# artpixls/ART

Measured on AMD Instinct MI355X. Metric: megapixels/sec end-to-end (AMaZE+FTblockDN+tone), 45 MP Bayer, higher is better.
Workload: dtype f32; 1 GPU; AMaZE + getImage/matrix + ImProcFunctions::denoise (chroma noise-curve map, FTblockDN wavelet shrinkage luma 40 / chroma 15 / gamma 1.7 + DCT detail recovery 50) + exposure 0.3 EV + tone curve STD, 8192x5464 Bayer RGGB fp32, 1 frame per GPU per step (BASELINE configs[2]); frame=8192x5464, lanes_per_gpu=1, parallelism=frame-per-gpu x1, completion_records=1, completion_via=single process

## Files before the change

### art_amd/csrc/detail.hip

```cpp
#include <hip/hip_runtime.h>
#include "devmath.h"
#include "devsleef.h"
#include "dct64.h"
#include "kernels.h"

namespace artgpu {

namespace {
constexpr int TS = 64, OFF = 25, BLKRAD = 1;
constexpr int NXCD = 8;
__device__ __forceinline__ int reflect(int v, int n)
{
    if (v < 0) return -v < n - 1 ? -v : n - 1;
    if (v >= n) return 2 * n - 2 - v > 0 ? 2 * n - 2 - v : 0;
    return v;
}
}

template <int RAD>
__global__ void __launch_bounds__(64) detail_blocks_kernel(DetailArgs a)
{
    constexpr int XR = 4;
    __shared__ float B[TS + XR][TS + 1];
    const int lane = threadIdx.x;
    const int wk = (a.numblox_W + NXCD - 1) / NXCD;
    const int xcd = blockIdx.x % NXCD, idx = blockIdx.x / NXCD;
    const int vblk = idx / wk, hblk = xcd * wk + (idx - vblk * wk);
    if (hblk >= a.numblox_W) return;
    const int blk = vblk * a.numblox_W + hblk;
    const int top = (vblk - BLKRAD) * OFF, left = (hblk - BLKRAD) * OFF;
    constexpr int rad = RAD;
    float x[TS];

    {
        const int cc = reflect(left + lane, a.w);
#pragma unroll
        for (int i = 0; i < TS; ++i) {
            const int rr = reflect(top + i, a.h);
            const size_t o = (size_t)rr * a.w + cc;
            x[i] = a.tm_in[i * TS + lane] * (a.Lin[o] - a.L[o]);
        }
    }
    lee_fwd<TS>(x);
#pragma unroll
    for (int k = 0; k < TS; ++k) B[k][lane] = 2.f * x[k];
    __syncthreads();
#pragma unroll
    for (int j = 0; j < TS; ++j) x[j] = B[lane][j];
    lee_fwd<TS>(x);
#pragma unroll
    for (int m = 0; m < TS; ++m) x[m] = 2.f * x[m];
    {
        int len = rad + 1;
        float tempval = fabsf(x[0]);
#pragma unroll
        for (int q = 1; q <= rad; q++) tempval += fabsf(x[q]);
        tempval /= len;
        B[lane][0] = tempval;
#pragma unroll
        for (int col = 1; col <= rad; col++) {
            tempval = (tempval * len + fabsf(x[col + rad])) / (len + 1);
            B[lane][col] = tempval;
            len++;
        }
        const float rlen = 1.f / (float)len;
#pragma unroll
        for (int col = rad + 1; col < TS - rad; col++) {
            tempval = tempval + (fabsf(x[col + rad]) - fabsf(x[col - rad - 1])) * rlen;
            B[lane][col] = tempval;
        }
#pragma unroll
        for (int col = TS - rad; col < TS; col++) {
            tempval = (tempval * len - fabsf(x[col - rad - 1])) / (len - 1);
            B[lane][col] = tempval;
            len--;
        }
    }
    __syncthreads();
    {
        float lenf = (float)(rad + 1);
        float tv = B[0][lane];
#pragma unroll
        for (int i = 1; i <= rad; i++) tv = tv + B[i][lane];
        tv = tv / lenf;
        const bool colin = (left + lane) >= 0 && (left + lane) < a.w;
        const float inv_hi = 1.f / a.detail_hi, inv_lo = 1.f / a.detail_lo;
        auto emit = [&](int row, float tvr) {
            const bool rowin = (top + row) >= 0 && (top + row) < a.h;
            float factor = (rowin && colin) ? a.detail_hi : a.detail_lo;
            const float rfac = (rowin && colin) ? inv_hi : inv_lo;
            const bool masked = a.mask && rowin && colin;
            if (masked) {
                const float d = a.params_Ldetail * a.mask[(size_t)(top + row) * a.w + left + lane];
                const float t = static_cast<float>((100. - d) * (100. - d) + 50. * (100. - d)) * TS * 0.5f;
                factor = t * t;
            }
            (void)factor; (void)rfac;
            const int slot = row > rad ? row - rad - 1 : TS + row;
#ifdef DETAIL_EXACT_DIV
            B[slot][lane] = 1.0f - __expf(-sqr(tvr) / factor);
#else
            if (a.mask) B[slot][lane] = 1.0f - __expf(masked ? -sqr(tvr) / factor : -sqr(tvr) * rfac);
            else B[slot][lane] = 1.0f - __expf(-sqr(tvr) * rfac);
#endif
        };
        emit(0, tv);
#pragma unroll
        for (int row = 1; row <= rad; ++row) {
            const float lenp1 = lenf + 1.f;
            tv = (tv * lenf + B[row + rad][lane]) / lenp1;
            lenf = lenp1;
            emit(row, tv);
        }
        const float rlen = 1.f / lenf;
        constexpr int S0 = rad + 1, S1 = TS - rad, G = 8;
        constexpr int SG = S0 + (S1 - S0) / G * G;
#ifndef DETAIL_ROW_AT_A_TIME
#pragma unroll 1
        for (int r0 = S0; r0 < SG; r0 += G) {
            float hi[G], lo[G], tvs[G];
#pragma unroll
            for (int k = 0; k < G; ++k) { hi[k] = B[r0 + k + rad][lane]; lo[k] = B[r0 + k - rad - 1][lane]; }
#pragma unroll
            for (int k = 0; k < G; ++k) { tv = tv + (hi[k] - lo[k]) * rlen; tvs[k] = tv; }
#pragma unroll
            for (int k = 0; k < G; ++k) emit(r0 + k, tvs[k]);
        }
#pragma unroll 1
        for (int row = SG; row < S1; ++row) {
#else
#pragma unroll 1
        for (int row = S0; row < S1; ++row) {
#endif
            tv = tv + (B[row + rad][lane] - B[row - rad - 1][lane]) * rlen;
            emit(row, tv);
        }
#pragma unroll 1
        for (int row = S1; row < TS; ++row) {
            const float lenm1 = lenf - 1.f;
            tv = (tv * lenf - B[row - rad - 1][lane]) / lenm1;
            lenf = lenm1;
            emit(row, tv);
        }
    }
    __syncthreads();
    {
        const int slot = lane > rad ? lane - rad - 1 : TS + lane;
#pragma unroll
        for (int m = 0; m < TS; ++m) x[m] = x[m] * B[slot][m];
    }
    __syncthreads();
#pragma unroll
    for (int m = 1; m < TS; ++m) x[m] = 2.f * x[m];
    lee_inv<TS>(x);
#pragma unroll
    for (int j = 0; j < TS; ++j) B[lane][j] = x[j];
    __syncthreads();
    x[0] = B[0][lane];
#pragma unroll
    for (int k = 1; k < TS; ++k) x[k] = 2.f * B[k][lane];
    lee_inv<TS>(x);
    float *out = a.blocks + (size_t)blk * TS * TS;
#pragma unroll
    for (int i = 0; i < TS; ++i) out[i * TS + lane] = x[i];
}

__global__ void __launch_bounds__(1024) detail_gather_kernel(DetailArgs a)
{
    __shared__ float s_in[TS * TS], s_out[TS * TS];
    for (int k = threadIdx.x; k < TS * TS; k += 1024) { s_in[k] = a.tm_in[k]; s_out[k] = a.tm_out[k]; }
    __syncthreads();
    const float DCTnorm = 1.0f / (4 * TS * TS);
    const long long n = (long long)a.w * a.h;
#ifndef DETAIL_GATHER_LOOPS
    for (long long t = blockIdx.x * (long long)blockDim.x + threadIdx.x; t < n; t += (long long)gridDim.x * blockDim.x) {
        const int y = (int)(t / a.w), x = (int)(t - (long long)y * a.w);
        const int yc = y / OFF, xc = x / OFF, ry = y - yc * OFF, rx = x - xc * OFF;
        bool vs[3], hs[3];
        int iv[3], jh[3], vb[3], hb[3];
#pragma unroll
        for (int k = 0; k < 3; ++k) {
            vs[k] = k > 0 || (yc > 0 && ry < TS - 2 * OFF);
            hs[k] = k > 0 || (xc > 0 && rx < TS - 2 * OFF);
            iv[k] = vs[k] ? ry + 2 * OFF - OFF * k : ry;  vb[k] = vs[k] ? yc - 1 + k : yc + 1;
            jh[k] = hs[k] ? rx + 2 * OFF - OFF * k : rx;  hb[k] = hs[k] ? xc - 1 + k : xc + 1;
        }
        float blk[9], tmo[9], tmi[9];
#pragma unroll
        for (int s_ = 0; s_ < 3; ++s_)
#pragma unroll
            for (int t_ = 0; t_ < 3; ++t_) {
                const int m = iv[s_] * TS + jh[t_];
                blk[3 * s_ + t_] = a.blocks[((size_t)vb[s_] * a.numblox_W + hb[t_]) * TS * TS + m];
                tmo[3 * s_ + t_] = s_out[m];
                tmi[3 * s_ + t_] = s_in[m];
            }
        const float Lold = a.L[t];
// ... 1 lines not shown
#pragma unroll
        for (int s_ = 0; s_ < 3; ++s_)
#pragma unroll
            for (int t_ = 0; t_ < 3; ++t_) {
                const bool v = vs[s_] && hs[t_];
                const float ld = Ldetail + tmo[3 * s_ + t_] * blk[3 * s_ + t_] * DCTnorm, tw = totwt + tmi[3 * s_ + t_] * tmo[3 * s_ + t_];
                Ldetail = v ? ld : Ldetail;
                totwt = v ? tw : totwt;
            }
        a.L[t] = Lold + Ldetail / totwt;
    }
#else
    for (long long t = blockIdx.x * (long long)blockDim.x + threadIdx.x; t < n; t += (long long)gridDim.x * blockDim.x) {
        const int y = (int)(t / a.w), x = (int)(t - (long long)y * a.w);
        const int vb0 = max(0, y / OFF + BLKRAD - 2), vb1 = min(a.numblox_H - 1, y / OFF + BLKRAD);
        const int hb0 = max(0, x / OFF + BLKRAD - 2), hb1 = min(a.numblox_W - 1, x / OFF + BLKRAD);
        float Ldetail = 0.f, totwt = 0.f;
        for (int vblk = vb0; vblk <= vb1; ++vblk) {
            const int i = y - (vblk - BLKRAD) * OFF;
            if (i < 0 || i >= TS) continue;
            for (int hblk = hb0; hblk <= hb1; ++hblk) {
                const int j = x - (hblk - BLKRAD) * OFF;
                if (j < 0 || j >= TS) continue;
                const float tmo = s_out[i * TS + j];
                Ldetail += tmo * a.blocks[((size_t)vblk * a.numblox_W + hblk) * TS * TS + i * TS + j] * DCTnorm;
                totwt += s_in[i * TS + j] * tmo;
            }
        }
        a.L[t] += Ldetail / totwt;
    }
#endif
}

hipError_t launch_detail_blocks(const DetailArgs &a, hipStream_t s)
{
    const dim3 grid(NXCD * ((a.numblox_W + NXCD - 1) / NXCD) * a.numblox_H);
    switch (a.blur_rad) {
    case 1: hipLaunchKernelGGL(detail_blocks_kernel<1>, grid, dim3(64), 0, s, a); break;
    case 2: hipLaunchKernelGGL(detail_blocks_kernel<2>, grid, dim3(64), 0, s, a); break;
    case 3: hipLaunchKernelGGL(detail_blocks_kernel<3>, grid, dim3(64), 0, s, a); break;
    default: return hipErrorInvalidValue;
    }
    return hipGetLastError();
}
hipError_t launch_detail_gather(const DetailArgs &a, hipStream_t s)
{
    const long long n = (long long)a.w * a.h;
    const long long g = (n + 1023) / 1024;
    int dev = 0, cus = 256;
    if (hipGetDevice(&dev) == hipSuccess) (void)hipDeviceGetAttribute(&cus, hipDeviceAttributeMultiprocessorCount, dev);
    const long long cap = 2LL * cus;
    hipLaunchKernelGGL(detail_gather_kernel, dim3((int)(g < cap ? g : cap)), dim3(1024), 0, s, a);
    return hipGetLastError();
}

}
```

### art_amd/csrc/artgpu_api.hip

```cpp
#include <hip/hip_runtime.h>
#include <dlfcn.h>
#include <cmath>
#include <cstdio>
#include <cstdarg>
#include <cstring>
#include <new>
#include <string>
#include <thread>
#include <vector>
#include <algorithm>

#include "../../include/artgpu.h"
#include "kernels.h"

using namespace artgpu;

struct artgpu_ctx {
    int device = 0;
    hipStream_t stream = nullptr;
    hipStream_t aux = nullptr;
    hipEvent_t aux_ev[2] = {nullptr, nullptr};
    hipStream_t dn_stream[1] = {nullptr};
    hipEvent_t dn_ev[2] = {nullptr, nullptr};
    const float *gam_tab = nullptr; float gam_key[6] = {};
    int opt_lut_lds = 1;
    int opt_dn_streams = 0;
    int ccalc_nonneg = 0;
    int opt_dn_fused = 1;
    std::string err;
    int *fs_diag = nullptr;
    int opt_dn_debug_stall = -1;
    long opt_dn_wait_ms = 0;
    long long batch_px = 0;
    int dn_form = -1, dn_form_streak = 0;
    float *arena = nullptr;
    size_t arena_bytes = 0;
    static constexpr int NSTAGE = 8;
    float *stage[NSTAGE] = {};
    size_t stage_bytes[NSTAGE] = {};
    static constexpr int NPOOL = 64;
    float *pool[NPOOL] = {};
    size_t pool_bytes[NPOOL] = {};
    std::vector<artgpu_ctx *> lanes;
    int batch_lanes = 1;
    int frames_in_flight = 1;
    bool owns_stream = false;
    hipStream_t io_up = nullptr, io_down = nullptr;
    hipEvent_t io_ev[8] = {};
    int *io_host = nullptr;
    int io_host_cap = 0;
    int cu_reserve = 0;
    int opt_io_direct = -1;
    float fuse_pre = 0.f, fuse_post = 0.f;
    GetImageFuse fuse_gi = {};
    float fuse_exp_scale = 0.f, fuse_exp_black = 0.f;
    int fuse_exp_on = 0;
    int tail_exp_on = 0;
    float tail_exp_scale = 0.f, tail_exp_black = 0.f;
    float *bbox = nullptr;
    size_t bbox_bytes = 0;
    float *amz_lists = nullptr;
// ... 354 lines not shown
}

int artgpu_get_option(artgpu_ctx *ctx, const char *name, long *value)
{
    if (!ctx || !name || !value) return ARTGPU_EINVAL;
    const std::string n(name);
    if (n.rfind("amaze_counter", 0) == 0 && n.size() == 14 && n[13] >= '0' && n[13] <= '7') {
        if (!ctx->amz_lists || ctx->amz_nstream <= 0) { *value = 0; return ARTGPU_OK; }
        HIPCHK(ctx, hipSetDevice(ctx->device));
        HIPCHK(ctx, hipStreamSynchronize(ctx->stream));
        const size_t nfixed = (((size_t)ctx->amz_nstream + (1 + ctx->amz_narena) + (1 + ctx->amz_narena + ctx->amz_nstream) + 3) / 4) * 4;
        int v = 0;
        HIPCHK(ctx, hipMemcpy(&v, reinterpret_cast<int *>(ctx->amz_lists) + nfixed + 4 + 2 * (size_t)ctx->amz_nstream + (n[13] - '0'), sizeof(int), hipMemcpyDeviceToHost));
        *value = v;
        return ARTGPU_OK;
    }
    return fail(ctx, ARTGPU_EINVAL, "get_option: unknown option '%s'", name);
}

int artgpu_set_option(artgpu_ctx *ctx, const char *name, long value)
{
    if (!ctx || !name) return ARTGPU_EINVAL;
    const std::string n(name);
    if (n == "amaze_path") { if (value < 0 || value > 1) return fail(ctx, ARTGPU_EINVAL, "amaze_path: 0 or 1"); ctx->opt_amaze_path = (int)value; }
    else if (n == "amaze_split") ctx->opt_amaze_split = value != 0;
    else if (n == "amaze_overlap") ctx->opt_amaze_overlap = value != 0;
    else if (n == "amaze_grid") { if (value < 0) return fail(ctx, ARTGPU_EINVAL, "amaze_grid: >= 0"); ctx->opt_amaze_grid = (int)value; }
    else if (n == "amaze_zero_mask") ctx->opt_amaze_zero_mask = value;
    else if (n == "amaze_zero_frame") ctx->opt_amaze_zero_frame = (int)value;
    else if (n == "amaze_poison") ctx->opt_amaze_poison = (int)value;
    else if (n == "roctx") ctx->opt_roctx = value != 0;
    else if (n == "dn_streams") ctx->opt_dn_streams = value != 0;
    else if (n == "dn_fused") ctx->opt_dn_fused = (int)value;
    else if (n == "dn_debug_stall") ctx->opt_dn_debug_stall = (int)value;
    else if (n == "dn_wait_ms") ctx->opt_dn_wait_ms = value < 0 ? 0 : value;
    else if (n == "lut_lds") ctx->opt_lut_lds = value != 0;
    else if (n == "cu_reserve") { if (value < 0 || value > 4096) return fail(ctx, ARTGPU_EINVAL, "cu_reserve: 0 .. 4096"); ctx->cu_reserve = (int)value; }
    else if (n == "io_direct") { if (value < -1 || value > 4096) return fail(ctx, ARTGPU_EINVAL, "io_direct: -1 (automatic), 0 .. 4096 workgroups"); ctx->opt_io_direct = (int)value; }
    else if (n == "rcd_rows") { if (value != 4 && value != 8) return fail(ctx, ARTGPU_EINVAL, "rcd_rows: 4 or 8"); ctx->opt_rcd_rows = (int)value; }
    else return fail(ctx, ARTGPU_EINVAL, "set_option: unknown option '%s'", name);
    return ARTGPU_OK;
}

int artgpu_set_progress_callback(artgpu_ctx *ctx, artgpu_progress_fn fn, void *user)
{
    if (!ctx) return ARTGPU_EINVAL;
    ctx->progress_fn = fn;
    ctx->progress_user = user;
    return ARTGPU_OK;
}

int artgpu_enable_timing(artgpu_ctx *ctx, int enable)
{
    if (!ctx) return ARTGPU_EINVAL;
    ctx->timing = enable != 0;
    return ARTGPU_OK;
}

int artgpu_get_timings(const artgpu_ctx *ctx, artgpu_timings *out)
{
    if (!ctx || !out) return ARTGPU_EINVAL;
    *out = ctx->last;
    return ARTGPU_OK;
}

size_t artgpu_scratch_bytes(const artgpu_ctx *ctx)
// ... 944 lines not shown
            da.detail_lo = compute_detail(0.f);
            { const int br = int(3 / scale); da.blur_rad = br > 1 ? br : 1; }
            float *dtab;
            const bool fresh_dtab = ctx->pool[P_DCTTAB] == nullptr;
            if ((rc2 = pool_get(ctx, P_DCTTAB, 4 * 4096 * 4, &dtab))) return rc2;
            if ((rc2 = pool_get(ctx, P_BLOCKS, (size_t)da.numblox_W * da.numblox_H * 4096 * 4, &da.blocks))) return rc2;
            if (fresh_dtab) {
                std::vector<float> host(4 * 4096);
                float *tm_in = host.data(), *tm_out = tm_in + 4096, *ct = tm_out + 4096, *ctt = ct + 4096;
                const float epsilon = 0.001f / (64 * 64);
                const int border = 4;
                for (int i = 0; i < 64; ++i) {
                    const float i1 = std::abs((i > 32 ? i - 64 + 1 : i));
                    const float vmask = (i1 < border ? (float)0 + (std::sin((M_PI * i1) / (2 * border)) * std::sin((M_PI * i1) / (2 * border))) : 1.0f);
                    const float vmask2 = (i1 < 2 * border ? (std::sin((M_PI * i1) / (2 * border)) * std::sin((M_PI * i1) / (2 * border))) : 1.0f);
                    for (int j = 0; j < 64; ++j) {
                        const float j1 = std::abs((j > 32 ? j - 64 + 1 : j));
                        const double sj = std::sin((M_PI * j1) / (2 * border));
                        tm_in[i * 64 + j] = (vmask * (j1 < border ? sj * sj : 1.0f)) + epsilon;
                        tm_out[i * 64 + j] = (vmask2 * (j1 < 2 * border ? sj * sj : 1.0f)) + epsilon;
                        ct[i * 64 + j] = (float)std::cos(M_PI * (j + 0.5) * i / 64.0);
                        ctt[j * 64 + i] = ct[i * 64 + j];
                    }
                }
                hipError_t e = hipMemcpyAsync(dtab, host.data(), host.size() * 4, hipMemcpyHostToDevice, sL);
                if (e == hipSuccess) e = hipStreamSynchronize(sL);
                if (e != hipSuccess) {
                    (void)hipFree(ctx->pool[P_DCTTAB]); ctx->pool[P_DCTTAB] = nullptr; ctx->pool_bytes[P_DCTTAB] = 0;
                    return fail(ctx, ARTGPU_EHIP, "rgb_denoise: upload of the DCT tables failed: %s", hipGetErrorString(e));
                }
            }
            da.tm_in = dtab; da.tm_out = dtab + 4096; da.costab = dtab + 2 * 4096; da.costab_t = dtab + 3 * 4096;
            da.L = Lout; da.Lin = Lin;
            if (p->luminance_detail_threshold > 0) {
                float *dmask;
                if ((rc2 = pool_get(ctx, P_DMASK, n * 4, &dmask))) return rc2;
                const float amount = std::max(0.f, std::min(float(p->luminance_detail_threshold) / 100.f, 1.f));
                float *dm_scratch = tmp;
                if (!dm_scratch && (rc2 = pool_get(ctx, P_TMP, ((size_t)w * h + 2 * (size_t)(w / 4) * (h / 4)) * 4, &dm_scratch))) return rc2;
                if ((rc2 = detail_mask_dev(ctx, Lout, (size_t)w, dmask, w, h, 65535.f, 25.f, 10000.f, amount, (float)(25.f / scale), dm_scratch))) return rc2;
                da.mask = dmask; da.params_Ldetail = params_Ldetail;
            }
            if (sd != sL) {
                HIPCHK(ctx, hipEventRecord(ctx->dn_ev[0], sL));
                HIPCHK(ctx, hipStreamWaitEvent(sd, ctx->dn_ev[0], 0));
            }
            HIPCHK(ctx, launch_detail_blocks(da, sd));
            HIPCHK(ctx, launch_detail_gather(da, sd));
            if (sd != sL) HIPCHK(ctx, hipEventRecord(ctx->dn_ev[1], sd));
        }
        return ARTGPU_OK;
    };

    auto merged_pass = [&]() -> int {
        FusedShrinkArgs fa = {};
        fa.coef = Ld.bands; fa.coef_out = Lbands2; fa.coefC = Cdd[0].bands; fa.coefL = Ld.bands; fa.n = n2; fa.w = w2; fa.h = h2;
        fa.madL = madL; fa.madab = merged_mad ? mad + nsub : mad + 32; fa.mad_ch_stride = nsub;
        fa.noisevar = ccalc_dev; fa.noisevar_nonneg = ctx->ccalc_nonneg; fa.noisevar_const = noisevarL; fa.noisevar_scale = maxNoiseVarab;
        fa.noisevar_ab[0] = noisevar_abc[0]; fa.noisevar_ab[1] = noisevar_abc[1];
        fa.useNoiseCCurve = useNoiseCCurve ? 1 : 0;
        for (int l = 0; l < 10; ++l) fa.rad[l] = bl0.rad[l];
        fa.level0 = 0; fa.nsub = 3 * nsub; fa.nL = nsub; fa.nsub_ch = nsub; fa.diag = ctx->fs_diag; fa.wait_ticks = (long long)ctx->opt_dn_wait_ms * 100000LL; fa.stall_band = ctx->opt_dn_debug_stall < 0 ? -1 : ctx->opt_dn_debug_stall >> 16; fa.stall_strip = ctx->opt_dn_debug_stall < 0 ? -1 : ctx->opt_dn_debug_stall & 0xffff;
        HIPCHK(ctx, launch_shrink_blur(fa, fused_scratch, sL));
        return ARTGPU_OK;
    };
    if (merged) {
// ... 1450 lines not shown
}

namespace {
int batch_settle_scratch(artgpu_ctx *c, long long px, long long nxt)
{
    if (nxt < 0) nxt = c->batch_px;
    if (c->batch_px && 2 * px < c->batch_px && 2 * nxt < c->batch_px) {
        std::vector<artgpu_ctx *> keep;
        keep.swap(c->lanes);
        const int rc = artgpu_trim_scratch(c);
        keep.swap(c->lanes);
        if (rc) return rc;
        c->batch_px = 0;
    }
    if (px > c->batch_px) c->batch_px = px;
    return ARTGPU_OK;
}

int batch_prepare_lanes(artgpu_ctx *ctx, int L)
{
    HIPCHK(ctx, hipSetDevice(ctx->device));
    while ((int)ctx->lanes.size() < L - 1) {
        artgpu_ctx *peer = nullptr;
        int rc = artgpu_create(ctx->device, &peer);
        if (rc) return fail(ctx, rc, "batch_run: cannot create lane %d", (int)ctx->lanes.size() + 1);
        if (hipStreamCreateWithFlags(&peer->stream, hipStreamNonBlocking) != hipSuccess) { (void)artgpu_destroy(peer); return fail(ctx, ARTGPU_EHIP, "batch_run: stream"); }
        peer->owns_stream = true;
        ctx->lanes.push_back(peer);
    }
    for (artgpu_ctx *peer : ctx->lanes) {
        peer->curve_tail_kind = ctx->curve_tail_kind; peer->curve_tail_y = ctx->curve_tail_y; peer->curve_tail_pc = ctx->curve_tail_pc;
        peer->opt_amaze_path = ctx->opt_amaze_path; peer->opt_amaze_split = ctx->opt_amaze_split; peer->opt_amaze_overlap = ctx->opt_amaze_overlap; peer->opt_amaze_grid = ctx->opt_amaze_grid;
        peer->opt_amaze_zero_mask = ctx->opt_amaze_zero_mask; peer->opt_amaze_zero_frame = ctx->opt_amaze_zero_frame; peer->opt_amaze_poison = ctx->opt_amaze_poison;
        peer->opt_rcd_rows = ctx->opt_rcd_rows; peer->opt_roctx = ctx->opt_roctx; peer->opt_lut_lds = ctx->opt_lut_lds; peer->opt_dn_streams = ctx->opt_dn_streams; peer->opt_dn_fused = ctx->opt_dn_fused;
        peer->opt_dn_wait_ms = ctx->opt_dn_wait_ms; peer->opt_dn_debug_stall = ctx->opt_dn_debug_stall; peer->opt_io_direct = ctx->opt_io_direct;
        peer->progress_fn = ctx->progress_fn; peer->progress_user = ctx->progress_user;
        peer->frames_in_flight = L;
    }
    ctx->frames_in_flight = L;
    return ARTGPU_OK;
}
struct InFlightReset { artgpu_ctx *c; ~InFlightReset() { c->frames_in_flight = 1; for (artgpu_ctx *p : c->lanes) p->frames_in_flight = 1; } };

extern "C++" {
template <typename F>
int batch_on_lanes(artgpu_ctx *ctx, int L, F work)
{
    std::vector<int> rcs(L, ARTGPU_OK);
    std::vector<artgpu_ctx *> cs(L, ctx);
    for (int k = 1; k < L; ++k) cs[k] = ctx->lanes[k - 1];
    std::vector<std::thread> threads;
    for (int k = 1; k < L; ++k) threads.emplace_back([&rcs, &work, &cs, k]() { rcs[k] = work(cs[k], k); });
    rcs[0] = work(ctx, 0);
    for (std::thread &t : threads) t.join();
    for (int k = 0; k < L; ++k)
        if (rcs[k]) return fail(ctx, rcs[k], "batch_run: lane %d: %s", k, k == 0 ? ctx->err.c_str() : cs[k]->err.c_str());
    return ARTGPU_OK;
}
}
}

int artgpu_batch_run(artgpu_ctx *ctx, int nframes, const artgpu_plane *raws, const artgpu_pipeline_params *params, artgpu_rgb *outs)
{
    if (!ctx) return ARTGPU_EINVAL;
    if (nframes < 0 || (nframes && (!raws || !params || !outs))) return fail(ctx, ARTGPU_EINVAL, "batch_run: null argument");
    const int L = std::min(ctx->batch_lanes, nframes);
    auto px_of = [&](int f) { return (long long)raws[f].w * raws[f].h; };
// ... 240 lines not shown
```

### art_amd/csrc/kernels.h

```cpp
#pragma once
#include <hip/hip_runtime.h>
#include "paramcurve.h"
#include <vector>
#include <stddef.h>
#include <stdint.h>
#include <mutex>
#include <set>
#include <utility>

inline hipError_t dyn_lds_once(const void *fn, int bytes)
{
    static std::mutex m;
    static std::set<std::pair<const void *, int>> done;
    int dev = 0;
    hipError_t e = hipGetDevice(&dev);
    if (e != hipSuccess) return e;
    std::lock_guard<std::mutex> lk(m);
    if (done.count({fn, dev})) return hipSuccess;
    e = hipFuncSetAttribute(fn, hipFuncAttributeMaxDynamicSharedMemorySize, bytes);
    if (e == hipSuccess) done.insert({fn, dev});
    return e;
}

inline bool device_block_fits(int lds_bytes, int threads)
// ... 394 lines not shown
    float noisevar_ab[2];
    int useNoiseCCurve;
    int rad[10];
    int level0;
    int nsub;
    int nL;
    int nsub_ch;
    int mad_ch_stride;
    int nstrips;
    float *hand;
    int wpad;
    int *progress;
    int *ticket;
    int *diag;
    long long wait_ticks;
    int stall_band, stall_strip;
    long long *prof;
};
bool shrink_blur_supported(int w, int h, const int *rad, int level0, int nsub);
size_t shrink_blur_scratch_floats(int w, int h, int nsub, int maxr);
hipError_t launch_shrink_blur(FusedShrinkArgs a, float *scratch, hipStream_t s);

struct DetailArgs {
    float *L;
    const float *Lin;
    const float *tm_in, *tm_out;
    const float *costab, *costab_t;
    float *blocks;
    int w, h, numblox_W, numblox_H;
    float detail_hi, detail_lo;
    int blur_rad;
    const float *mask;
    float params_Ldetail;
};
hipError_t launch_detail_blocks(const DetailArgs &a, hipStream_t s);
hipError_t launch_detail_gather(const DetailArgs &a, hipStream_t s);

struct GuidedArgs {
    float *rgb[3];
    size_t stride;
    int W, H;
    int w, h;
    float *in[3];
    float *guide;
    float *chan[3];
    float *low[8];
    double ws1[3];
    float epsilon;
    int nch;
    float *q; size_t q_stride;
};
hipError_t launch_gf_prepare(const GuidedArgs &a, hipStream_t s);
hipError_t launch_gf_subsample(const GuidedArgs &a, hipStream_t s);
hipError_t launch_gf_ab(const GuidedArgs &a, hipStream_t s);
hipError_t launch_gf_finish(const GuidedArgs &a, hipStream_t s);
hipError_t launch_gf_finish_plain(const GuidedArgs &a, hipStream_t s);

struct MaskArgs {
    const float *src; size_t src_stride;
    float *L2, *m2;
    float *mask;
    int W, H, w4, h4;
    float scaling, threshold, ceiling, factor;
};
struct GaussArgs {
    float *img, *tmp;
// ... 44 lines not shown
```

Before: 4454 MP/s.

## Shrink detail-block LDS footprint with split transposes and two-part box filter

The detail DCT block kernel's shared buffer goes from 68x65 floats to 52x65. The two transposes now run in two 32-lane halves with float4 stores, and the separable box filter runs in two passes that share one ring-like buffer. Row offsets for the input gather are computed once per lane and broadcast with readlane, giving 32-bit byte offsets in place of per-row reflect and 64-bit index math. The aim is more resident workgroups per CU from lower LDS use and cheaper address arithmetic, at the cost of extra barriers and more complex slot indexing.

Result: no change. 4439 MP/s (-0.3%).

```diff
diff --git a/art_amd/csrc/detail.hip b/art_amd/csrc/detail.hip
--- a/art_amd/csrc/detail.hip
+++ b/art_amd/csrc/detail.hip
@@ -17,11 +17,32 @@
 }
 }
 
+__device__ __forceinline__ void transpose64(float *S, int lane, float (&v)[TS])
+{
+    constexpr int CS = TS + 4;
+    float y[TS];
+#pragma unroll
+    for (int half = 0; half < 2; ++half) {
+        if ((lane >> 5) == half) {
+#pragma unroll
+            for (int q = 0; q < TS / 4; ++q)
+                *reinterpret_cast<float4 *>(&S[(lane & 31) * CS + 4 * q]) = make_float4(v[4 * q], v[4 * q + 1], v[4 * q + 2], v[4 * q + 3]);
+        }
+        __syncthreads();
+#pragma unroll
+        for (int r = 0; r < TS / 2; ++r) y[half * (TS / 2) + r] = S[r * CS + lane];
+        __syncthreads();
+    }
+#pragma unroll
+    for (int r = 0; r < TS; ++r) v[r] = y[r];
+}
+
 template <int RAD>
 __global__ void __launch_bounds__(64) detail_blocks_kernel(DetailArgs a)
 {
-    constexpr int XR = 4;
-    __shared__ float B[TS + XR][TS + 1];
+    constexpr int NB = 52, LS = TS + 1;
+    constexpr int P = NB - 4;
+    __shared__ __attribute__((aligned(16))) float S[NB * LS];
     const int lane = threadIdx.x;
     const int wk = (a.numblox_W + NXCD - 1) / NXCD;
     const int xcd = blockIdx.x % NXCD, idx = blockIdx.x / NXCD;
@@ -34,55 +55,28 @@
 
     {
         const int cc = reflect(left + lane, a.w);
+        const int rbase = max(0, min(top, a.h - (TS + OFF + 1)));
+        const char *lin0 = reinterpret_cast<const char *>(a.Lin + (size_t)rbase * a.w), *l0 = reinterpret_cast<const char *>(a.L + (size_t)rbase * a.w);
+        const unsigned rowb = (unsigned)(reflect(top + lane, a.h) - rbase) * (unsigned)a.w * 4u, colb = (unsigned)cc * 4u;
 #pragma unroll
         for (int i = 0; i < TS; ++i) {
-            const int rr = reflect(top + i, a.h);
-            const size_t o = (size_t)rr * a.w + cc;
-            x[i] = a.tm_in[i * TS + lane] * (a.Lin[o] - a.L[o]);
+            const unsigned ob = (unsigned)__builtin_amdgcn_readlane((int)rowb, i) + colb;
+            x[i] = a.tm_in[i * TS + lane] * (*reinterpret_cast<const float *>(lin0 + ob) - *reinterpret_cast<const float *>(l0 + ob));
         }
     }
     lee_fwd<TS>(x);
 #pragma unroll
-    for (int k = 0; k < TS; ++k) B[k][lane] = 2.f * x[k];
-    __syncthreads();
-#pragma unroll
-    for (int j = 0; j < TS; ++j) x[j] = B[lane][j];
+    for (int k = 0; k < TS; ++k) x[k] = 2.f * x[k];
+    transpose64(S, lane, x);
     lee_fwd<TS>(x);
 #pragma unroll
     for (int m = 0; m < TS; ++m) x[m] = 2.f * x[m];
     {
-        int len = rad + 1;
-        float tempval = fabsf(x[0]);
-#pragma unroll
-        for (int q = 1; q <= rad; q++) tempval += fabsf(x[q]);
-        tempval /= len;
-        B[lane][0] = tempval;
-#pragma unroll
-        for (int col = 1; col <= rad; col++) {
-            tempval = (tempval * len + fabsf(x[col + rad])) / (len + 1);
-            B[lane][col] = tempval;
-            len++;
-        }
-        const float rlen = 1.f / (float)len;
-#pragma unroll
-        for (int col = rad + 1; col < TS - rad; col++) {
-            tempval = tempval + (fabsf(x[col + rad]) - fabsf(x[col - rad - 1])) * rlen;
-            B[lane][col] = tempval;
-        }
-#pragma unroll
-        for (int col = TS - rad; col < TS; col++) {
-            tempval = (tempval * len - fabsf(x[col - rad - 1])) / (len - 1);
-            B[lane][col] = tempval;
-            len--;
-        }
-    }
-    __syncthreads();
-    {
-        float lenf = (float)(rad + 1);
-        float tv = B[0][lane];
-#pragma unroll
-        for (int i = 1; i <= rad; i++) tv = tv + B[i][lane];
-        tv = tv / lenf;
+        constexpr int WA = P - rad;
+        constexpr int S0 = rad + 1, S1 = TS - rad, G = 8;
+        static_assert(P + rad + 1 <= NB && TS - P + (TS - WA) <= WA - rad - 1, "the two parts overlap in the buffer");
+        auto nslot = [](int row) { return row < P ? row : row - P; };
+        auto fslot = [](int row) { return row <= rad ? P + row : row < WA ? row - rad - 1 : TS - P + row - WA; };
         const bool colin = (left + lane) >= 0 && (left + lane) < a.w;
         const float inv_hi = 1.f / a.detail_hi, inv_lo = 1.f / a.detail_lo;
         auto emit = [&](int row, float tvr) {
@@ -96,69 +90,101 @@
                 factor = t * t;
             }
             (void)factor; (void)rfac;
-            const int slot = row > rad ? row - rad - 1 : TS + row;
+            float *dst = &S[fslot(row) * LS + lane];
 #ifdef DETAIL_EXACT_DIV
-            B[slot][lane] = 1.0f - __expf(-sqr(tvr) / factor);
+            *dst = 1.0f - __expf(-sqr(tvr) / factor);
 #else
-            if (a.mask) B[slot][lane] = 1.0f - __expf(masked ? -sqr(tvr) / factor : -sqr(tvr) * rfac);
-            else B[slot][lane] = 1.0f - __expf(-sqr(tvr) * rfac);
+            if (a.mask) *dst = 1.0f - __expf(masked ? -sqr(tvr) / factor : -sqr(tvr) * rfac);
+            else *dst = 1.0f - __expf(-sqr(tvr) * rfac);
 #endif
         };
-        emit(0, tv);
-#pragma unroll
-        for (int row = 1; row <= rad; ++row) {
-            const float lenp1 = lenf + 1.f;
-            tv = (tv * lenf + B[row + rad][lane]) / lenp1;
-            lenf = lenp1;
-            emit(row, tv);
-        }
-        const float rlen = 1.f / lenf;
-        constexpr int S0 = rad + 1, S1 = TS - rad, G = 8;
-        constexpr int SG = S0 + (S1 - S0) / G * G;
-#ifndef DETAIL_ROW_AT_A_TIME
-#pragma unroll 1
-        for (int r0 = S0; r0 < SG; r0 += G) {
-            float hi[G], lo[G], tvs[G];
-#pragma unroll
-            for (int k = 0; k < G; ++k) { hi[k] = B[r0 + k + rad][lane]; lo[k] = B[r0 + k - rad - 1][lane]; }
-#pragma unroll
-            for (int k = 0; k < G; ++k) { tv = tv + (hi[k] - lo[k]) * rlen; tvs[k] = tv; }
-#pragma unroll
-            for (int k = 0; k < G; ++k) emit(r0 + k, tvs[k]);
-        }
-#pragma unroll 1
-        for (int row = SG; row < S1; ++row) {
-#else
-#pragma unroll 1
-        for (int row = S0; row < S1; ++row) {
-#endif
-            tv = tv + (B[row + rad][lane] - B[row - rad - 1][lane]) * rlen;
-            emit(row, tv);
-        }
-#pragma unroll 1
-        for (int row = S1; row < TS; ++row) {
-            const float lenm1 = lenf - 1.f;
-            tv = (tv * lenf - B[row - rad - 1][lane]) / lenm1;
-            lenf = lenm1;
-            emit(row, tv);
-        }
-    }
-    __syncthreads();
-    {
-        const int slot = lane > rad ? lane - rad - 1 : TS + lane;
-#pragma unroll
-        for (int m = 0; m < TS; ++m) x[m] = x[m] * B[slot][m];
-    }
-    __syncthreads();
+        float lenf = (float)(rad + 1), tv = 0.f;
+#pragma unroll 1
+        for (int part = 0; part < 2; ++part) {
+            if (part == 0 ? lane < P : lane >= P) {
+                float *N = &S[nslot(lane) * LS];
+                int len = rad + 1;
+                float tempval = fabsf(x[0]);
+#pragma unroll
+                for (int q = 1; q <= rad; q++) tempval += fabsf(x[q]);
+                tempval /= len;
+                N[0] = tempval;
+#pragma unroll
+                for (int col = 1; col <= rad; col++) {
+                    tempval = (tempval * len + fabsf(x[col + rad])) / (len + 1);
+                    N[col] = tempval;
+                    len++;
+                }
+                const float rlen = 1.f / (float)len;
+#pragma unroll
+                for (int col = rad + 1; col < TS - rad; col++) {
+                    tempval = tempval + (fabsf(x[col + rad]) - fabsf(x[col - rad - 1])) * rlen;
+                    N[col] = tempval;
+                }
+#pragma unroll
+                for (int col = TS - rad; col < TS; col++) {
+                    tempval = (tempval * len - fabsf(x[col - rad - 1])) / (len - 1);
+                    N[col] = tempval;
+                    len--;
+                }
+            }
+            __syncthreads();
+            if (part == 0) {
+                tv = S[lane];
+#pragma unroll
+                for (int i = 1; i <= rad; i++) tv = tv + S[i * LS + lane];
+                tv = tv / lenf;
+                emit(0, tv);
+#pragma unroll
+                for (int row = 1; row <= rad; ++row) {
+                    const float lenp1 = lenf + 1.f;
+                    tv = (tv * lenf + S[(row + rad) * LS + lane]) / lenp1;
+                    lenf = lenp1;
+                    emit(row, tv);
+                }
+            }
+            const float rlen = 1.f / lenf;
+            const int ra = part == 0 ? S0 : WA, rb = part == 0 ? WA : S1;
+            int r0 = ra;
+#pragma unroll 1
+            for (; r0 + G <= rb; r0 += G) {
+                float hi[G], lo[G], tvs[G];
+#pragma unroll
+                for (int k = 0; k < G; ++k) { hi[k] = S[nslot(r0 + k + rad) * LS + lane]; lo[k] = S[nslot(r0 + k - rad - 1) * LS + lane]; }
+#pragma unroll
+                for (int k = 0; k < G; ++k) { tv = tv + (hi[k] - lo[k]) * rlen; tvs[k] = tv; }
+#pragma unroll
+                for (int k = 0; k < G; ++k) emit(r0 + k, tvs[k]);
+            }
+#pragma unroll 1
+            for (int row = r0; row < rb; ++row) {
+                tv = tv + (S[nslot(row + rad) * LS + lane] - S[nslot(row - rad - 1) * LS + lane]) * rlen;
+                emit(row, tv);
+            }
+            if (part == 1) {
+#pragma unroll 1
+                for (int row = S1; row < TS; ++row) {
+                    const float lenm1 = lenf - 1.f;
+                    tv = (tv * lenf - S[nslot(row - rad - 1) * LS + lane]) / lenm1;
+                    lenf = lenm1;
+                    emit(row, tv);
+                }
+            }
+            __syncthreads();
+            if (part == 0 ? lane < WA : lane >= WA) {
+                const float *F = &S[fslot(lane) * LS];
+#pragma unroll
+                for (int m = 0; m < TS; ++m) x[m] = x[m] * F[m];
+            }
+            __syncthreads();
+        }
+    }
 #pragma unroll
     for (int m = 1; m < TS; ++m) x[m] = 2.f * x[m];
     lee_inv<TS>(x);
-#pragma unroll
-    for (int j = 0; j < TS; ++j) B[lane][j] = x[j];
-    __syncthreads();
-    x[0] = B[0][lane];
-#pragma unroll
-    for (int k = 1; k < TS; ++k) x[k] = 2.f * B[k][lane];
+    transpose64(S, lane, x);
+#pragma unroll
+    for (int k = 1; k < TS; ++k) x[k] = 2.f * x[k];
     lee_inv<TS>(x);
     float *out = a.blocks + (size_t)blk * TS * TS;
 #pragma unroll
```

## Trim unused DCT detail blocks, fast-path interior loads, and row-wise detail gather

Applied to the files above, without the earlier changes.

The detail-recovery block kernel now skips the last row and column of blocks, which the gather never reads. Interior blocks get a fast load path with 32-bit offsets, compressed window coefficients and shrink factors specialised at compile time. A new gather kernel has each wave process a 64-wide strip of rows, hoists per-column block offsets and reads precomputed total weights from LDS for interior pixels. The old paths remain behind a dn_detail_plain option; the price is more code paths and new bounds logic that could be wrong at the edges.

Result: faster. 4429 MP/s before, 4505 MP/s after (median of 6 runs) (+1.7%).

```diff
diff --git a/art_amd/csrc/artgpu_api.hip b/art_amd/csrc/artgpu_api.hip
--- a/art_amd/csrc/artgpu_api.hip
+++ b/art_amd/csrc/artgpu_api.hip
@@ -27,6 +27,7 @@
     int opt_dn_streams = 0;
     int ccalc_nonneg = 0;
     int opt_dn_fused = 1;
+    int opt_dn_detail_plain = 0;
     std::string err;
     int *fs_diag = nullptr;
     int opt_dn_debug_stall = -1;
@@ -447,6 +448,7 @@
     else if (n == "roctx") ctx->opt_roctx = value != 0;
     else if (n == "dn_streams") ctx->opt_dn_streams = value != 0;
     else if (n == "dn_fused") ctx->opt_dn_fused = (int)value;
+    else if (n == "dn_detail_plain") { if (value < 0 || value > 3) return fail(ctx, ARTGPU_EINVAL, "dn_detail_plain: 0 .. 3"); ctx->opt_dn_detail_plain = (int)value; }
     else if (n == "dn_debug_stall") ctx->opt_dn_debug_stall = (int)value;
     else if (n == "dn_wait_ms") ctx->opt_dn_wait_ms = value < 0 ? 0 : value;
     else if (n == "lut_lds") ctx->opt_lut_lds = value != 0;
@@ -1457,6 +1459,7 @@
             }
             da.tm_in = dtab; da.tm_out = dtab + 4096; da.costab = dtab + 2 * 4096; da.costab_t = dtab + 3 * 4096;
             da.L = Lout; da.Lin = Lin;
+            da.plain = ctx->opt_dn_detail_plain == 1 ? 3 : ctx->opt_dn_detail_plain == 2 ? 1 : ctx->opt_dn_detail_plain == 3 ? 2 : 0;
             if (p->luminance_detail_threshold > 0) {
                 float *dmask;
                 if ((rc2 = pool_get(ctx, P_DMASK, n * 4, &dmask))) return rc2;
@@ -2973,7 +2976,7 @@
         peer->curve_tail_kind = ctx->curve_tail_kind; peer->curve_tail_y = ctx->curve_tail_y; peer->curve_tail_pc = ctx->curve_tail_pc;
         peer->opt_amaze_path = ctx->opt_amaze_path; peer->opt_amaze_split = ctx->opt_amaze_split; peer->opt_amaze_overlap = ctx->opt_amaze_overlap; peer->opt_amaze_grid = ctx->opt_amaze_grid;
         peer->opt_amaze_zero_mask = ctx->opt_amaze_zero_mask; peer->opt_amaze_zero_frame = ctx->opt_amaze_zero_frame; peer->opt_amaze_poison = ctx->opt_amaze_poison;
-        peer->opt_rcd_rows = ctx->opt_rcd_rows; peer->opt_roctx = ctx->opt_roctx; peer->opt_lut_lds = ctx->opt_lut_lds; peer->opt_dn_streams = ctx->opt_dn_streams; peer->opt_dn_fused = ctx->opt_dn_fused;
+        peer->opt_rcd_rows = ctx->opt_rcd_rows; peer->opt_roctx = ctx->opt_roctx; peer->opt_lut_lds = ctx->opt_lut_lds; peer->opt_dn_streams = ctx->opt_dn_streams; peer->opt_dn_fused = ctx->opt_dn_fused; peer->opt_dn_detail_plain = ctx->opt_dn_detail_plain;
         peer->opt_dn_wait_ms = ctx->opt_dn_wait_ms; peer->opt_dn_debug_stall = ctx->opt_dn_debug_stall; peer->opt_io_direct = ctx->opt_io_direct;
         peer->progress_fn = ctx->progress_fn; peer->progress_user = ctx->progress_user;
         peer->frames_in_flight = L;
diff --git a/art_amd/csrc/detail.hip b/art_amd/csrc/detail.hip
--- a/art_amd/csrc/detail.hip
+++ b/art_amd/csrc/detail.hip
@@ -1,4 +1,5 @@
 #include <hip/hip_runtime.h>
+#include <type_traits>
 #include "devmath.h"
 #include "devsleef.h"
 #include "dct64.h"
@@ -8,6 +9,7 @@
 
 namespace {
 constexpr int TS = 64, OFF = 25, BLKRAD = 1;
+constexpr int XR = 4;
 constexpr int NXCD = 8;
 __device__ __forceinline__ int reflect(int v, int n)
 {
@@ -17,22 +19,27 @@
 }
 }
 
-template <int RAD>
-__global__ void __launch_bounds__(64) detail_blocks_kernel(DetailArgs a)
-{
-    constexpr int XR = 4;
-    __shared__ float B[TS + XR][TS + 1];
+#ifdef DETAIL_PHASE_MARKS
+#define DETAIL_PHASE(name) asm volatile("; detail-phase " name)
+#else
+#define DETAIL_PHASE(name)
+#endif
+
+template <int RAD, bool INSIDE, bool MASKED>
+__device__ __forceinline__ void detail_shrink_factors(const DetailArgs &a, float (*B)[TS + 1], int top, int left, int lane);
+
+template <int RAD, bool TRIM>
+__device__ __forceinline__ void detail_block(const DetailArgs &a, float (*B)[TS + 1], const int vblk, const int hblk)
+{
     const int lane = threadIdx.x;
-    const int wk = (a.numblox_W + NXCD - 1) / NXCD;
-    const int xcd = blockIdx.x % NXCD, idx = blockIdx.x / NXCD;
-    const int vblk = idx / wk, hblk = xcd * wk + (idx - vblk * wk);
-    if (hblk >= a.numblox_W) return;
     const int blk = vblk * a.numblox_W + hblk;
     const int top = (vblk - BLKRAD) * OFF, left = (hblk - BLKRAD) * OFF;
     constexpr int rad = RAD;
+    const bool inside = TRIM && a.inside32 && top >= 0 && top + TS <= a.h && left >= 0 && left + TS <= a.w;
     float x[TS];
 
-    {
+    DETAIL_PHASE("load");
+    if (!TRIM) {
         const int cc = reflect(left + lane, a.w);
 #pragma unroll
         for (int i = 0; i < TS; ++i) {
@@ -40,7 +47,35 @@
             const size_t o = (size_t)rr * a.w + cc;
             x[i] = a.tm_in[i * TS + lane] * (a.Lin[o] - a.L[o]);
         }
-    }
+    } else {
+        constexpr int MB = 4;
+        const float tm_mid = a.tm_in[(TS / 2) * TS + lane];
+        float tm_end[2 * MB];
+#pragma unroll
+        for (int i = 0; i < MB; ++i) { tm_end[i] = a.tm_in[i * TS + lane]; tm_end[MB + i] = a.tm_in[(TS - MB + i) * TS + lane]; }
+        auto tm = [&](int i) { return i < MB ? tm_end[i] : i >= TS - MB ? tm_end[i - (TS - 2 * MB)] : tm_mid; };
+        if (inside) {
+            DETAIL_PHASE("load-inside");
+            const char *pin = (const char *)(a.Lin + ((size_t)top * a.w + left)), *pl = (const char *)(a.L + ((size_t)top * a.w + left));
+            const unsigned pitch = (unsigned)a.w * 4u;
+            unsigned o = (unsigned)lane * 4u;
+#pragma unroll
+            for (int i = 0; i < TS; ++i) {
+                x[i] = tm(i) * (*(const float *)(pin + o) - *(const float *)(pl + o));
+                o += pitch;
+            }
+        } else {
+            DETAIL_PHASE("load-border");
+            const int cc = reflect(left + lane, a.w);
+#pragma unroll
+            for (int i = 0; i < TS; ++i) {
+                const int rr = reflect(top + i, a.h);
+                const size_t o = (size_t)rr * a.w + cc;
+                x[i] = tm(i) * (a.Lin[o] - a.L[o]);
+            }
+        }
+    }
+    DETAIL_PHASE("forward");
     lee_fwd<TS>(x);
 #pragma unroll
     for (int k = 0; k < TS; ++k) B[k][lane] = 2.f * x[k];
@@ -50,6 +85,7 @@
     lee_fwd<TS>(x);
 #pragma unroll
     for (int m = 0; m < TS; ++m) x[m] = 2.f * x[m];
+    DETAIL_PHASE("rowblur");
     {
         int len = rad + 1;
         float tempval = fabsf(x[0]);
@@ -77,19 +113,53 @@
         }
     }
     __syncthreads();
+    DETAIL_PHASE("factors");
+    if (!inside) detail_shrink_factors<RAD, false, false>(a, B, top, left, lane);
+    else if (a.mask) detail_shrink_factors<RAD, true, true>(a, B, top, left, lane);
+    else detail_shrink_factors<RAD, true, false>(a, B, top, left, lane);
+    DETAIL_PHASE("inverse");
+    __syncthreads();
+    {
+        const int slot = lane > rad ? lane - rad - 1 : TS + lane;
+#pragma unroll
+        for (int m = 0; m < TS; ++m) x[m] = x[m] * B[slot][m];
+    }
+    __syncthreads();
+#pragma unroll
+    for (int m = 1; m < TS; ++m) x[m] = 2.f * x[m];
+    lee_inv<TS>(x);
+#pragma unroll
+    for (int j = 0; j < TS; ++j) B[lane][j] = x[j];
+    __syncthreads();
+    x[0] = B[0][lane];
+#pragma unroll
+    for (int k = 1; k < TS; ++k) x[k] = 2.f * B[k][lane];
+    lee_inv<TS>(x);
+    float *out = a.blocks + (size_t)blk * TS * TS;
+#pragma unroll
+    for (int i = 0; i < TS; ++i) out[i * TS + lane] = x[i];
+    DETAIL_PHASE("end");
+}
+
+template <int RAD, bool INSIDE, bool MASKED>
+__device__ __forceinline__ void detail_shrink_factors(const DetailArgs &a, float (*B)[TS + 1], const int top, const int left, const int lane)
+{
+    constexpr int rad = RAD;
+    if constexpr (INSIDE) DETAIL_PHASE("factors-inside"); else DETAIL_PHASE("factors-border");
     {
         float lenf = (float)(rad + 1);
         float tv = B[0][lane];
 #pragma unroll
         for (int i = 1; i <= rad; i++) tv = tv + B[i][lane];
         tv = tv / lenf;
-        const bool colin = (left + lane) >= 0 && (left + lane) < a.w;
+        const bool colin = INSIDE || ((left + lane) >= 0 && (left + lane) < a.w);
         const float inv_hi = 1.f / a.detail_hi, inv_lo = 1.f / a.detail_lo;
         auto emit = [&](int row, float tvr) {
-            const bool rowin = (top + row) >= 0 && (top + row) < a.h;
+            const bool rowin = INSIDE || ((top + row) >= 0 && (top + row) < a.h);
             float factor = (rowin && colin) ? a.detail_hi : a.detail_lo;
             const float rfac = (rowin && colin) ? inv_hi : inv_lo;
-            const bool masked = a.mask && rowin && colin;
+            const bool anymask = INSIDE ? MASKED : a.mask != nullptr;
+            const bool masked = anymask && rowin && colin;
             if (masked) {
                 const float d = a.params_Ldetail * a.mask[(size_t)(top + row) * a.w + left + lane];
                 const float t = static_cast<float>((100. - d) * (100. - d) + 50. * (100. - d)) * TS * 0.5f;
@@ -100,7 +170,7 @@
 #ifdef DETAIL_EXACT_DIV
             B[slot][lane] = 1.0f - __expf(-sqr(tvr) / factor);
 #else
-            if (a.mask) B[slot][lane] = 1.0f - __expf(masked ? -sqr(tvr) / factor : -sqr(tvr) * rfac);
+            if (anymask) B[slot][lane] = 1.0f - __expf(masked ? -sqr(tvr) / factor : -sqr(tvr) * rfac);
             else B[slot][lane] = 1.0f - __expf(-sqr(tvr) * rfac);
 #endif
         };
@@ -143,26 +213,29 @@
             emit(row, tv);
         }
     }
-    __syncthreads();
-    {
-        const int slot = lane > rad ? lane - rad - 1 : TS + lane;
-#pragma unroll
-        for (int m = 0; m < TS; ++m) x[m] = x[m] * B[slot][m];
-    }
-    __syncthreads();
-#pragma unroll
-    for (int m = 1; m < TS; ++m) x[m] = 2.f * x[m];
-    lee_inv<TS>(x);
-#pragma unroll
-    for (int j = 0; j < TS; ++j) B[lane][j] = x[j];
-    __syncthreads();
-    x[0] = B[0][lane];
-#pragma unroll
-    for (int k = 1; k < TS; ++k) x[k] = 2.f * B[k][lane];
-    lee_inv<TS>(x);
-    float *out = a.blocks + (size_t)blk * TS * TS;
-#pragma unroll
-    for (int i = 0; i < TS; ++i) out[i * TS + lane] = x[i];
+}
+
+template <int RAD>
+__global__ void __launch_bounds__(64) detail_blocks_kernel(DetailArgs a)
+{
+    __shared__ float B[TS + XR][TS + 1];
+    const int wk = (a.numblox_W + NXCD - 1) / NXCD;
+    const int xcd = blockIdx.x % NXCD, idx = blockIdx.x / NXCD;
+    const int vblk = idx / wk, hblk = xcd * wk + (idx - vblk * wk);
+    if (hblk >= a.numblox_W) return;
+    detail_block<RAD, false>(a, B, vblk, hblk);
+}
+
+template <int RAD>
+__global__ void __launch_bounds__(64) detail_blocks_trim_kernel(DetailArgs a)
+{
+    __shared__ float B[TS + XR][TS + 1];
+    const int nw = a.numblox_W - 1;
+    const int wk = (nw + NXCD - 1) / NXCD;
+    const int xcd = blockIdx.x % NXCD, idx = blockIdx.x / NXCD;
+    const int vblk = idx / wk, hblk = xcd * wk + (idx - vblk * wk);
+    if (hblk >= nw) return;
+    detail_block<RAD, true>(a, B, vblk, hblk);
 }
 
 __global__ void __launch_bounds__(1024) detail_gather_kernel(DetailArgs a)
@@ -230,24 +303,133 @@
 #endif
 }
 
-hipError_t launch_detail_blocks(const DetailArgs &a, hipStream_t s)
-{
-    const dim3 grid(NXCD * ((a.numblox_W + NXCD - 1) / NXCD) * a.numblox_H);
+__global__ void __launch_bounds__(1024) detail_gather_rows_kernel(DetailArgs a)
+{
+    __shared__ float s_in[TS * TS], s_out[TS * TS], s_tw[OFF * OFF];
+    for (int k = threadIdx.x; k < TS * TS; k += 1024) { s_in[k] = a.tm_in[k]; s_out[k] = a.tm_out[k]; }
+    __syncthreads();
+    constexpr int NEAR = TS - 2 * OFF;
+    for (int k = threadIdx.x; k < OFF * OFF; k += 1024) {
+        const int ry = k / OFF, rx = k - ry * OFF;
+        float totwt = 0.f;
+#pragma unroll
+        for (int s_ = 0; s_ < 3; ++s_)
+#pragma unroll
+            for (int t_ = 0; t_ < 3; ++t_) {
+                const bool v = (s_ > 0 || ry < NEAR) && (t_ > 0 || rx < NEAR);
+                const int m = v ? (ry + 2 * OFF - OFF * s_) * TS + rx + 2 * OFF - OFF * t_ : 0;
+                const float tw = totwt + s_in[m] * s_out[m];
+                totwt = v ? tw : totwt;
+            }
+        s_tw[k] = totwt;
+    }
+    __syncthreads();
+    const float DCTnorm = 1.0f / (4 * TS * TS);
+    const int wave = __builtin_amdgcn_readfirstlane(threadIdx.x >> 6), lane = threadIdx.x & 63;
+    const int ncx = (a.w + 63) / 64, ncy = (a.h + OFF - 1) / OFF;
+    const int nunits = ncx * ncy;
+    const size_t brow = (size_t)a.numblox_W * TS * TS;
+    for (int u = wave * gridDim.x + blockIdx.x; u < nunits; u += 16 * gridDim.x) {
+        const int yc = __builtin_amdgcn_readfirstlane(u / ncx), cx = u - yc * ncx;
+        const int x = cx * 64 + lane;
+        const bool xin = x < a.w;
+        const int xx = xin ? x : a.w - 1;
+        const int xc = xx / OFF, rx = xx - xc * OFF;
+        const bool h0 = xc > 0 && rx < NEAR;
+        int jh[3];
+        unsigned co[3];
+#pragma unroll
+        for (int t_ = 0; t_ < 3; ++t_) {
+            const bool hs = t_ > 0 || h0;
+            jh[t_] = hs ? rx + 2 * OFF - OFF * t_ : rx;
+            co[t_] = (unsigned)((hs ? xc - 1 + t_ : xc + 1) * (TS * TS) + jh[t_]) * 4u;
+        }
+        const int rows = min(OFF, a.h - yc * OFF);
+        const int rows0 = yc > 0 ? min(rows, NEAR) : 0;
+        const unsigned lo = (unsigned)(xx - cx * 64) * 4u;
+        char *Lrow = (char *)(a.L + ((size_t)yc * OFF * a.w + (size_t)cx * 64));
+        const char *b0 = (const char *)(a.blocks + ((size_t)(yc > 0 ? yc - 1 : 0) * brow + 2 * OFF * TS));
+        const char *b1 = (const char *)(a.blocks + ((size_t)yc * brow + OFF * TS));
+        const char *b2 = (const char *)(a.blocks + (size_t)(yc + 1) * brow);
+        const bool whole = yc > 0 && xc > 0;
+        auto row = [&](const int ry, auto above) {
+            constexpr bool V0 = decltype(above)::value;
+            constexpr int S0 = V0 ? 0 : 1;
+            const size_t ro = (size_t)ry * TS * 4;
+            const char *bs[3] = {b0 + ro, b1 + ro, b2 + ro};
+            float blk[9], tmo[9];
+#pragma unroll
+            for (int s_ = S0; s_ < 3; ++s_)
+#pragma unroll
+                for (int t_ = 0; t_ < 3; ++t_) {
+                    blk[3 * s_ + t_] = *(const float *)(bs[s_] + co[t_]);
+                    tmo[3 * s_ + t_] = s_out[(ry + 2 * OFF - OFF * s_) * TS + jh[t_]];
+                }
+            const float Lold = *(const float *)(Lrow + (size_t)ry * a.w * 4 + lo);
+            float Ldetail = 0.f;
+#pragma unroll
+            for (int s_ = S0; s_ < 3; ++s_)
+#pragma unroll
+                for (int t_ = 0; t_ < 3; ++t_) {
+                    const float ld = Ldetail + tmo[3 * s_ + t_] * blk[3 * s_ + t_] * DCTnorm;
+                    Ldetail = (t_ > 0 || h0) ? ld : Ldetail;
+                }
+            float totwt;
+            if (whole) totwt = s_tw[ry * OFF + rx];
+            else {
+                totwt = 0.f;
+#pragma unroll
+                for (int s_ = S0; s_ < 3; ++s_)
+#pragma unroll
+                    for (int t_ = 0; t_ < 3; ++t_) {
+                        const int m = (ry + 2 * OFF - OFF * s_) * TS + jh[t_];
+                        const float tw = totwt + s_in[m] * s_out[m];
+                        totwt = (t_ > 0 || h0) ? tw : totwt;
+                    }
+            }
+            if (xin) *(float *)(Lrow + (size_t)ry * a.w * 4 + lo) = Lold + Ldetail / totwt;
+        };
+        for (int ry = 0; ry < rows0; ++ry) row(ry, std::true_type());
+        for (int ry = rows0; ry < rows; ++ry) row(ry, std::false_type());
+    }
+}
+
+hipError_t launch_detail_blocks(const DetailArgs &a_, hipStream_t s)
+{
+    DetailArgs a = a_;
+    if (a.plain & 1) {
+        const dim3 grid(NXCD * ((a.numblox_W + NXCD - 1) / NXCD) * a.numblox_H);
+        switch (a.blur_rad) {
+        case 1: hipLaunchKernelGGL(detail_blocks_kernel<1>, grid, dim3(64), 0, s, a); break;
+        case 2: hipLaunchKernelGGL(detail_blocks_kernel<2>, grid, dim3(64), 0, s, a); break;
+        case 3: hipLaunchKernelGGL(detail_blocks_kernel<3>, grid, dim3(64), 0, s, a); break;
+        default: return hipErrorInvalidValue;
+        }
+        return hipGetLastError();
+    }
+    a.inside32 = (long long)a.w * a.h <= (1LL << 30);
+    const dim3 grid(NXCD * ((a.numblox_W - 1 + NXCD - 1) / NXCD) * (a.numblox_H - 1));
     switch (a.blur_rad) {
-    case 1: hipLaunchKernelGGL(detail_blocks_kernel<1>, grid, dim3(64), 0, s, a); break;
-    case 2: hipLaunchKernelGGL(detail_blocks_kernel<2>, grid, dim3(64), 0, s, a); break;
-    case 3: hipLaunchKernelGGL(detail_blocks_kernel<3>, grid, dim3(64), 0, s, a); break;
+    case 1: hipLaunchKernelGGL(detail_blocks_trim_kernel<1>, grid, dim3(64), 0, s, a); break;
+    case 2: hipLaunchKernelGGL(detail_blocks_trim_kernel<2>, grid, dim3(64), 0, s, a); break;
+    case 3: hipLaunchKernelGGL(detail_blocks_trim_kernel<3>, grid, dim3(64), 0, s, a); break;
     default: return hipErrorInvalidValue;
     }
     return hipGetLastError();
 }
 hipError_t launch_detail_gather(const DetailArgs &a, hipStream_t s)
 {
-    const long long n = (long long)a.w * a.h;
-    const long long g = (n + 1023) / 1024;
     int dev = 0, cus = 256;
     if (hipGetDevice(&dev) == hipSuccess) (void)hipDeviceGetAttribute(&cus, hipDeviceAttributeMultiprocessorCount, dev);
     const long long cap = 2LL * cus;
+    const long long units = ((long long)a.w + 63) / 64 * (((long long)a.h + OFF - 1) / OFF);
+    if (!(a.plain & 2) && (long long)a.numblox_W * TS * TS * 4 < (1LL << 32) && units + 16 * cap < (1LL << 31)) {
+        const long long g = (units + 15) / 16;
+        hipLaunchKernelGGL(detail_gather_rows_kernel, dim3((int)(g < cap ? g : cap)), dim3(1024), 0, s, a);
+        return hipGetLastError();
+    }
+    const long long n = (long long)a.w * a.h;
+    const long long g = (n + 1023) / 1024;
     hipLaunchKernelGGL(detail_gather_kernel, dim3((int)(g < cap ? g : cap)), dim3(1024), 0, s, a);
     return hipGetLastError();
 }
diff --git a/art_amd/csrc/kernels.h b/art_amd/csrc/kernels.h
--- a/art_amd/csrc/kernels.h
+++ b/art_amd/csrc/kernels.h
@@ -450,6 +450,8 @@
     int blur_rad;
     const float *mask;
     float params_Ldetail;
+    int plain;
+    int inside32;
 };
 hipError_t launch_detail_blocks(const DetailArgs &a, hipStream_t s);
 hipError_t launch_detail_gather(const DetailArgs &a, hipStream_t s);
```
